# ZikangXiong/mobrob

Hardware: AMD Instinct MI355X
Metric: env-steps/sec (whole node), doggo PPO (higher is better)
Workload: dtype f32

## Files before the change

include/mobrob_ppo.h:

```cpp
#ifndef MOBROB_PPO_H
#define MOBROB_PPO_H

#include <stddef.h>
#include <stdint.h>

#ifdef __cplusplus
extern "C" {
#endif

#define MOBROB_PPO_ABI_VERSION 3
enum { MOBROB_ACT_TANH = 0, MOBROB_ACT_RELU = 1, MOBROB_ACT_ELU = 2, MOBROB_ACT_LEAKY_RELU = 3, MOBROB_ACT_SIGMOID = 4,
       MOBROB_ACT_SOFTPLUS = 5, MOBROB_ACT_SOFTSIGN = 6, MOBROB_ACT_HARDTANH = 7, MOBROB_ACT_RELU6 = 8, MOBROB_ACT_SILU = 9,
       MOBROB_ACT_GELU = 10, MOBROB_ACT_MISH = 11, MOBROB_ACT_COUNT = 12 };

enum {
  MOBROB_OK = 0,
  MOBROB_ERR_INVALID = -1,
  MOBROB_ERR_HIP = -2,
  MOBROB_ERR_STATE = -3,
  MOBROB_ERR_NO_DEVICE = -4
};

typedef struct mobrob_ppo_engine mobrob_ppo_engine_t;

// ... 459 lines not shown
  MOBROB_BUF_TERMINAL_OBS = 15,
  MOBROB_BUF_TERMINAL_VALUES = 16,
  MOBROB_BUF_TRUNCATED = 17,
  MOBROB_BUF_ENV_STATE = 18,
  MOBROB_BUF_GRAD_EXCHANGE = 19,
  MOBROB_BUF_SDE_NOISE = 20,
  MOBROB_BUF_COUNT = 21
};
int mobrob_ppo_buffer_info(mobrob_ppo_engine_t* e, int32_t which, void** ptr_dev, size_t* bytes);
int mobrob_ppo_read_buffer(mobrob_ppo_engine_t* e, int32_t which, void* host_out, size_t bytes);
int mobrob_ppo_write_buffer(mobrob_ppo_engine_t* e, int32_t which, const void* host_in, size_t bytes);
int mobrob_ppo_mark_rollout_ready(mobrob_ppo_engine_t* e);

int mobrob_ppo_x3_mode(const mobrob_ppo_engine_t* e);
int mobrob_ppo_update_mode(const mobrob_ppo_engine_t* e);

int mobrob_ppo_explained_variance(mobrob_ppo_engine_t* e, double* out);

int mobrob_ppo_compute_gae(mobrob_ppo_engine_t* e);

int mobrob_ppo_feistel_permutation(mobrob_ppo_engine_t* e, int64_t n, uint64_t key, int64_t* out);

enum {
  MOBROB_K_ACT = 0,
  MOBROB_K_GAE = 1,
  MOBROB_K_TRAIN_GRAD = 2,
  MOBROB_K_APPLY = 3,
  MOBROB_K_ENV = 4,
  MOBROB_K_GRAD_REDUCE = 5,
  MOBROB_K_ALLREDUCE = 6,
// ... 10 lines not shown
```

mobrob_amd/_lib.py:

```python
from __future__ import annotations

import ctypes as C
import os

_HERE = os.path.dirname(os.path.abspath(__file__))
LIB_PATH = os.environ.get("MOBROB_PPO_LIB") or os.path.join(_HERE, "libmobrob_ppo.so")
ABI_VERSION = 3

OK, ERR_INVALID, ERR_HIP, ERR_STATE, ERR_NO_DEVICE = 0, -1, -2, -3, -4

BUF = dict(obs=0, actions=1, rewards=2, episode_starts=3, values=4, log_probs=5, advantages=6, returns=7,
           params=8, grads=9, advstat=10, last_values=11, last_dones=12, clipped_actions=13, episode_start_state=14,
           terminal_obs=15, terminal_values=16, truncated=17, env_state=18, grad_exchange=19, sde_noise=20)
HYPER = dict(learning_rate=0, clip_range=1, clip_range_vf=2, target_kl=3, ent_coef=4, vf_coef=5, epoch_kernel=6)
KERNEL_IDS = dict(act=0, gae=1, train_grad=2, apply=3, env=4, grad_reduce=5, allreduce=6)


class Config(C.Structure):
    _fields_ = [
        ("abi_version", C.c_int32), ("obs_dim", C.c_int32), ("act_dim", C.c_int32),
        ("pi_hidden", C.c_int32 * 2), ("vf_hidden", C.c_int32 * 2),
        ("n_envs", C.c_int32), ("n_steps", C.c_int32), ("batch_size", C.c_int32), ("n_epochs", C.c_int32),
        ("gamma", C.c_double), ("gae_lambda", C.c_double), ("clip_range", C.c_double), ("ent_coef", C.c_double),
        ("vf_coef", C.c_double), ("max_grad_norm", C.c_double), ("learning_rate", C.c_double),
# ... 216 lines not shown
                                                   C.POINTER(C.c_uint16), C.c_int32, C.POINTER(C.c_int32), C.c_int32, _U8,
                                                   C.POINTER(C.c_int32), C.POINTER(C.c_int32)]),
    "mobrob_ppo_plan_assign": (C.c_int, [_P, C.POINTER(PlanSpec), C.POINTER(WallsC), C.POINTER(HazardsC), C.POINTER(HazardFramesC),
                                         C.POINTER(PlanTime), C.c_int32, C.c_int32, _F, _F, C.POINTER(C.c_int32), _F, C.POINTER(C.c_int32),
                                         _I64, C.POINTER(C.c_int32), _I64, _I64, C.POINTER(C.c_int32), C.POINTER(C.c_int32)]),
    "mobrob_ppo_sde_reset_noise": (C.c_int, [_P]),
    "mobrob_ppo_sde_set_noise": (C.c_int, [_P, _F]),
    "mobrob_ppo_buffer_info": (C.c_int, [_P, C.c_int32, C.POINTER(_P), C.POINTER(C.c_size_t)]),
    "mobrob_ppo_read_buffer": (C.c_int, [_P, C.c_int32, _P, C.c_size_t]),
    "mobrob_ppo_write_buffer": (C.c_int, [_P, C.c_int32, _P, C.c_size_t]),
    "mobrob_ppo_mark_rollout_ready": (C.c_int, [_P]),
    "mobrob_ppo_compute_gae": (C.c_int, [_P]),
    "mobrob_ppo_explained_variance": (C.c_int, [_P, C.POINTER(C.c_double)]),
    "mobrob_ppo_x3_mode": (C.c_int, [_P]),
    "mobrob_ppo_update_mode": (C.c_int, [_P]),
    "mobrob_ppo_feistel_permutation": (C.c_int, [_P, C.c_int64, C.c_uint64, _I64]),
    "mobrob_ppo_profile_enable": (C.c_int, [_P, C.c_int32]),
    "mobrob_ppo_profile_read": (C.c_int, [_P, C.POINTER(C.c_double), _I64]),
}

ALLREDUCE_FN = C.CFUNCTYPE(C.c_int, C.c_void_p, C.c_void_p, C.c_size_t, C.c_int32, C.c_void_p)

_lib = None


class EngineError(RuntimeError):
    pass


def load():
# ... 24 lines not shown
```

mobrob_amd/csrc/engine.hip:

```cpp
#include <hip/hip_runtime.h>
#include <rccl/rccl.h>
#include <dlfcn.h>

#include <algorithm>
#include <atomic>
#include <thread>
#include <cmath>
#include <cstdarg>
#include <cstdio>
#include <climits>
#include <cstring>
#include <ctime>
#include <cstdlib>
#include <string>
#include <vector>

#ifdef MOBROB_POISON_LDS
namespace mobrob {
__global__ __launch_bounds__(1024) void k_poison_lds() {
  extern __shared__ unsigned poison_words[];
  volatile unsigned* w = poison_words;
  for (int i = threadIdx.x; i < 160 * 256; i += 1024) w[i] = 0xFFFFFFFFu;
}
inline void poison_lds(hipStream_t st) {
// ... 158 lines not shown
  ncclComm_t comm = nullptr;
  int64_t allreduce_calls = 0, allreduce_bytes = 0;
  struct OneShot {
    char* xbuf = nullptr;
    size_t payload = 0;
    char* peer[kOneShotMaxRanks] = {nullptr};
    int world = 0, rank = -1;
    bool ready = false;
    unsigned long long seq = 0;
    int* error = nullptr;
    long long timeout_ticks = 0;
  } oneshot;
  double* norm_rec_sum = nullptr; int* norm_rec_t = nullptr; int* fold_idx_dev = nullptr;
  int fold_start[kMaxTensors + 1] = {0};
  bool use_norm_records = false;
  bool epoch_kernel_on = true;
  unsigned* epoch_bar = nullptr;
  float* epoch_consts = nullptr;
  int* epoch_idx = nullptr;
  char* epoch_stage = nullptr;
  int* epoch_err_host = nullptr;
  hipEvent_t epoch_ev = nullptr;
  int last_update_mode = 0;
  float* epoch_snap = nullptr;
  int rollout64_tile_max = 256;
  int pair64_min_tiles = 65;
  int split64_max_tiles = 64;
  float *Xg = nullptr, *actg = nullptr, *lpg = nullptr, *advg = nullptr, *retg = nullptr, *oldvg = nullptr;
  float *hp[kMaxHidden] = {nullptr}, *hv[kMaxHidden] = {nullptr}, *mu = nullptr, *vout = nullptr;
  float *dmu = nullptr, *dv = nullptr, *dzp[kMaxHidden] = {nullptr}, *dzv[kMaxHidden] = {nullptr};
// ... 43 lines not shown
  bool plan_clear_lds_set = false;
  char* plan_time_buf = nullptr;
  size_t plan_time_bytes = 0;
  bool plan_time_lds_set = false;
  char* plan_team_buf = nullptr;
  size_t plan_team_bytes = 0;
  bool plan_team_lds_set = false;
  bool plan_team_smooth_lds_set = false;
  bool plan_team_rounds_lds_set = false;
  bool plan_assign_lds_set = false;
};

namespace {

int check_async_error(mobrob_ppo_engine* e);

constexpr size_t kArenaAlign = 256;

template <typename Tp>
int dalloc(mobrob_ppo_engine* e, Tp** p, size_t count) {
  const size_t bytes = (std::max<size_t>(count, 1) * sizeof(Tp) + kArenaAlign - 1) / kArenaAlign * kArenaAlign;
  if (e->plan_only) {
    e->arena_used += bytes;
    *p = nullptr;
    return MOBROB_OK;
  }
  if (e->arena_used + bytes > e->arena_bytes)
    return fail(MOBROB_ERR_INVALID, "device arena too small: need more than %zu bytes", e->arena_bytes);
  void* q = e->arena + e->arena_used;
  e->arena_used += bytes;
// ... 199 lines not shown
    c.D = e->D; c.Dp = e->Dp;
    hipLaunchKernelGGL(k_pack_chain, dim3(FH * FH / 256, 2), dim3(256), 0, e->stream, c);
  }
}

void repack(mobrob_ppo_engine* e) {
  auto pad = [&](const float* src, float* dst, int r, int c, int rp, int cp) {
    hipLaunchKernelGGL(k_pad_rows, dim3(cdiv(rp * cp, 256)), dim3(256), 0, e->stream, src, dst, r, c, rp, cp);
  };
  pad(Pp(e, T_PW1), e->pW1p, e->H1, e->D, e->H1, e->Dp);
  pad(Pp(e, T_VW1), e->vW1p, e->G1, e->D, e->G1, e->Dp);
  pad(Pp(e, T_AW), e->aWp, e->A, e->HL, e->Ap, e->HL);
  pad(Pp(e, T_VW), e->vWp, 1, e->GL, 8, e->GL);
  fused_repack(e->fused, e->params, e->offs, e->stream);
  pack_x3_all(e);
}

void forward_generic(mobrob_ppo_engine* e, const float* X, int rows, bool want_pi, float* mu_out, bool want_v,
                     float* v_out, bool keep_z = false) {
  GemmQueue qp, qv;
  if (want_pi) {
    linear_fwd(e, X, e->Dp, e->pW1p, e->Dp, Pp(e, e->tPB[0]), e->hp[0], e->Hp[0], rows, e->Hp[0], e->Dp, true, keep_z ? e->dzp[0] : nullptr, &qp);
    for (int l = 1; l < e->Lp; ++l)
      linear_fwd(e, e->hp[l - 1], e->Hp[l - 1], Pp(e, e->tPW[l]), e->Hp[l - 1], Pp(e, e->tPB[l]), e->hp[l], e->Hp[l], rows, e->Hp[l], e->Hp[l - 1], true,
                 keep_z ? e->dzp[l] : nullptr, &qp);
    linear_fwd(e, e->hp[e->Lp - 1], e->HL, e->aWp, e->HL, Pp(e, T_AB), mu_out, e->Ap, rows, e->A, e->HL, false, nullptr, &qp);
  }
  if (want_v) {
    linear_fwd(e, X, e->Dp, e->vW1p, e->Dp, Pp(e, e->tVB[0]), e->hv[0], e->Hv[0], rows, e->Hv[0], e->Dp, true, keep_z ? e->dzv[0] : nullptr, &qv);
    for (int l = 1; l < e->Lv; ++l)
      linear_fwd(e, e->hv[l - 1], e->Hv[l - 1], Pp(e, e->tVW[l]), e->Hv[l - 1], Pp(e, e->tVB[l]), e->hv[l], e->Hv[l], rows, e->Hv[l], e->Hv[l - 1], true,
                 keep_z ? e->dzv[l] : nullptr, &qv);
    linear_fwd(e, e->hv[e->Lv - 1], e->GL, e->vWp, e->GL, Pp(e, T_VB), v_out, 1, rows, 1, e->GL, false, nullptr, &qv);
  }
  run_queues(e, qp, qv, 1);
}

void forward(mobrob_ppo_engine* e, const float* X, int rows, bool want_pi, float* mu_out, bool want_v, float* v_out) {
  if (e->fused.enabled && fused_forward(e->fused, X, rows, want_pi, mu_out, e->Ap, want_v, v_out, e->stream)) return;
  forward_generic(e, X, rows, want_pi, mu_out, want_v, v_out);
}

int value_net_width_sum(const mobrob_ppo_engine* e) {
  int s = 0;
  for (int l = 0; l < e->Lv; ++l) s += e->Hv[l];
  return s;
}
ValueNetArgs value_net_args(mobrob_ppo_engine* e) {
  ValueNetArgs vn{};
  for (int l = 0; l < e->Lv; ++l) { vn.W[l] = Pp(e, e->tVW[l]); vn.b[l] = Pp(e, e->tVB[l]); vn.G[l] = e->Hv[l]; }
  vn.Wv = Pp(e, T_VW); vn.bv = Pp(e, T_VB);
  vn.L = e->Lv; vn.act = e->cfg.activation; vn.width_sum = value_net_width_sum(e);
  return vn;
// ... 19 lines not shown
void sde_resample(mobrob_ppo_engine* e, int r0, int n, uint32_t draw, const uint32_t* draw_base, bool single) {
  const int HLA = e->HL * e->A, per = cdiv(HLA, 4);
  hipLaunchKernelGGL(k_sde_resample, dim3(cdiv((n + (single ? 1 : 0)) * per, 256)), dim3(256), 0, e->stream, Pp(e, T_LOGSTD), HLA, e->A, e->sde_mode, r0, n,
                     eps_seed(e) ^ 0x5DE5DE5DE5DE5DEull, draw, draw_base, e->sde_E, single ? e->sde_E1 : (float*)nullptr);
}

void sde_variance(mobrob_ppo_engine* e, int rows, bool fresh_table, float* lat2 = nullptr) {
  if (fresh_table)
    hipLaunchKernelGGL(k_sde_std2, dim3(cdiv(e->HL * e->A, 256)), dim3(256), 0, e->stream, Pp(e, T_LOGSTD), e->HL, e->A, e->sde_mode, e->sde_S2);
  hipLaunchKernelGGL(k_sde_var, dim3(cdiv(rows, 4)), dim3(256), 0, e->stream, e->hp[e->Lp - 1], e->HL, e->sde_S2, rows, e->HL, e->A, e->sde_var, e->Ap,
                     lat2);
}

void act_rows(mobrob_ppo_engine* e, int t, int r0, int n, const float* eps_dev_or_null, uint32_t draw,
              const uint32_t* draw_base, float* clip_out = nullptr) {
  ProfScope ps(e, MOBROB_K_ACT);
  if (!clip_out) clip_out = e->clip_act + (size_t)r0 * e->A;
  const size_t row = (size_t)t * e->N + r0;
  const float* X = e->obs + row * e->Dp;
  if (e->fused.enabled) {
    FusedActArgs a{};
    a.X = X; a.rows = n; a.row0 = r0; a.want_pi = 1; a.want_v = 1; a.mu = nullptr; a.ldmu = e->Ap;
    a.v = e->values + row; a.sample = 1; a.A = e->A; a.log_std = Pp(e, T_LOGSTD); a.eps = eps_dev_or_null;
    a.seed = eps_seed(e); a.draw = draw; a.draw_base = draw_base; a.lo = (float)e->cfg.action_low; a.hi = (float)e->cfg.action_high;
    a.act_raw = e->actions + row * e->A; a.act_clip = clip_out; a.logp = e->logp + row;
    fused_launch_act(e->fused, a, e->stream);
    return;
  }
  forward(e, X, n, true, e->mu, true, e->values + row);
  if (e->sde) {
// ... 62 lines not shown
StatsArgs stats_args(const mobrob_ppo_engine* e) {
  StatsArgs st{};
  st.loss_sums = e->grads + e->P; st.log_std = e->params + e->offs[T_LOGSTD]; st.n_act = e->A; st.sde = e->sde;
  st.ent_coef = (float)e->cfg.ent_coef; st.vf_coef = (float)e->cfg.vf_coef;
  return st;
}
int fused_carve_packs(mobrob_ppo_engine* e) {
  FusedState& f = e->fused;
  const int H = f.H;
  const size_t nW1 = (size_t)(H / 32) * (e->Dp / 8) * 256, nW2 = (size_t)(H / 32) * (H / 8) * 256;
  const size_t nW3f = (size_t)(H / 8) * 256, nW3b = (size_t)(H / 32) * 4 * 256;
  const size_t nW3h = (size_t)(H / 16) * 256;
  const size_t per_net = nW1 + 2 * nW2 + nW3f + nW3h + nW3b + 2 * H;
  f.packed_floats = 2 * per_net;
  CHK(dalloc(e, &f.packed, f.packed_floats));
  const int head_bias[2] = {T_AB, T_VB};
  for (int n = 0; n < 2; ++n) {
    float* p = f.packed + n * per_net;
    f.net[n].W1f = reinterpret_cast<const f32x4*>(p); p += nW1;
    f.net[n].W2f = reinterpret_cast<const f32x4*>(p); p += nW2;
    f.net[n].W3f = reinterpret_cast<const f32x4*>(p); p += nW3f;
    f.net[n].W2b = reinterpret_cast<const f32x4*>(p); p += nW2;
    f.net[n].W3b = reinterpret_cast<const f32x4*>(p); p += nW3b;
    f.net[n].b1s = p; p += H;
    f.net[n].b2s = p; p += H;
    f.net[n].W3h = reinterpret_cast<const f32x4*>(p); p += nW3h;
    f.net[n].b3 = e->params + e->offs[head_bias[n]];
    f.net[n].head = n == 0 ? e->A : 1;
    f.net[n].W1x = nullptr; f.net[n].W2x = nullptr; f.net[n].W2bx = nullptr;
    f.net[n].W1c = nullptr; f.net[n].W2c = nullptr; f.net[n].W2bc = nullptr; f.net[n].W3c = nullptr; f.net[n].W3bc = nullptr;
// ... 13 lines not shown
    f.lds_act_bytes = fused64_lds_bytes(e->Dp);
    CHK(dalloc(e, &e->epoch_bar, 1024));
    CHK(dalloc(e, &e->epoch_snap, (size_t)3 * e->P));
    CHK(dalloc(e, &e->epoch_consts, (size_t)2 * e->nmb));
    CHK(dalloc(e, &e->epoch_idx, (size_t)e->nmb));
  } else {
    f.slab_floats = slab_size(e->Dp);
    CHK(dalloc(e, &f.slabs, (size_t)f.max_grid * f.slab_floats));
    if (e->cfg.forward_x3 && e->cfg.activation == MOBROB_ACT_TANH && !env_switched_off("MOBROB_NO_X3")) {
      for (int n = 0; n < 2; ++n) {
        unsigned* w1 = nullptr; unsigned* w2 = nullptr; unsigned* w2b = nullptr;
        CHK(dalloc(e, &w1, (size_t)(H / 32) * (e->Dp / 16) * 192 * 4));
        CHK(dalloc(e, &w2, (size_t)(H / 32) * (H / 16) * 192 * 4));
        CHK(dalloc(e, &w2b, (size_t)(H / 32) * (H / 16) * 192 * 4));
        f.net[n].W1x = w1; f.net[n].W2x = w2; f.net[n].W2bx = w2b;
      }
      f.train_x3 = e->A <= 16 && e->Dp != 48 && !env_switched_off("MOBROB_NO_TRAIN_X3");
      f.train_chain = f.train_x3 && !env_switched_off("MOBROB_NO_CHAIN");
      if (f.train_chain) {
        const int K1 = (e->Dp + 31) / 32;
        for (int n = 0; n < 2; ++n) {
          unsigned* w1 = nullptr; unsigned* w2 = nullptr; unsigned* w2b = nullptr; float* w3 = nullptr; float* w3b = nullptr;
          CHK(dalloc(e, &w1, (size_t)K1 * 16 * 768));
          CHK(dalloc(e, &w2, (size_t)8 * 16 * 768));
          CHK(dalloc(e, &w2b, (size_t)8 * 16 * 768));
          CHK(dalloc(e, &w3, (size_t)16 * 64 * 4));
          CHK(dalloc(e, &w3b, (size_t)16 * 64 * 4));
          f.net[n].W1c = w1; f.net[n].W2c = w2; f.net[n].W2bc = w2b; f.net[n].W3c = w3; f.net[n].W3bc = w3b;
        }
        f.lds_chain_bytes = chain_lds_bytes(e->Dp);
      }
    }
    CHK(dalloc(e, &f.train_rec, (size_t)e->N * e->T * train_rec_width(e->A)));
    f.lds_bytes = fused_lds_bytes(e->Dp);
    f.lds_act_bytes = fused_lds_act_bytes(e->Dp);
  }
  return dalloc(e, &f.stamps, 32);
}
int build_norm_record_tables(mobrob_ppo_engine* e) {
  const FusedState& f = e->fused;
  const int nb = cdiv(f.slab_floats, 256);
  CHK(dalloc(e, &e->norm_rec_sum, (size_t)2 * nb * kNormRec));
  CHK(dalloc(e, &e->norm_rec_t, (size_t)2 * nb * kNormRec));
// ... 353 lines not shown
  e->stats_cap = std::max(64, 4 * e->nmb * cfg->n_epochs);
  e->chunk_table.clear();
  for (int tt = 0; tt < e->ntens; ++tt)
    for (int s0 = e->offs[tt]; s0 < e->offs[tt + 1]; s0 += 4096)
      e->chunk_table.push_back(NormChunk{tt, s0, std::min(s0 + 4096, e->offs[tt + 1]), 0});
  e->nchunks = (int)e->chunk_table.size();
  if (e->nchunks > 256) return fail(MOBROB_ERR_INVALID, "parameter vector too large for the norm chunk table (%d chunks)", e->nchunks);
  return MOBROB_OK;
}

int engine_alloc(mobrob_ppo_engine* e) {
  const size_t P = e->P, N = e->N, T = e->T, Dp = e->Dp, A = e->A, Bl = std::min(e->Bl, e->N * e->T), R = e->rows_max;
  CHK(dalloc(e, &e->params, P)); CHK(dalloc(e, &e->grads, P + 8)); CHK(dalloc(e, &e->m, P)); CHK(dalloc(e, &e->v, P));
  CHK(dalloc(e, &e->pW1p, (size_t)e->H1 * Dp)); CHK(dalloc(e, &e->vW1p, (size_t)e->G1 * Dp));
  CHK(dalloc(e, &e->aWp, (size_t)e->Ap * e->HL)); CHK(dalloc(e, &e->vWp, (size_t)8 * e->GL));
  CHK(dalloc(e, &e->obs, (T + 1) * N * Dp)); CHK(dalloc(e, &e->actions, T * N * A));
  CHK(dalloc(e, &e->rewards, T * N)); CHK(dalloc(e, &e->es, T * N)); CHK(dalloc(e, &e->values, (T + 1) * N));
  e->last_values = e->values + T * N;
  CHK(dalloc(e, &e->logp, T * N)); CHK(dalloc(e, &e->adv, T * N)); CHK(dalloc(e, &e->ret, T * N));
  CHK(dalloc(e, &e->last_dones, N)); CHK(dalloc(e, &e->prev_dones, N));
  CHK(dalloc(e, &e->dones_tmp, N)); CHK(dalloc(e, &e->clip_act, N * A)); CHK(dalloc(e, &e->rew_tmp, N));
  CHK(dalloc(e, &e->term_obs, N * Dp)); CHK(dalloc(e, &e->term_val, N)); CHK(dalloc(e, &e->eps_dev, R * A));
  CHK(dalloc(e, &e->trunc_dev, N)); CHK(dalloc(e, &e->dones_u8, N)); CHK(dalloc(e, &e->ep_len, N)); CHK(dalloc(e, &e->ep_len2, N)); CHK(dalloc(e, &e->ctr_dev, 2));
  CHK(dalloc(e, &e->rows, T * N)); CHK(dalloc(e, &e->perm_dev, T * N)); CHK(dalloc(e, &e->advstat, (size_t)e->nmb * 4)); CHK(dalloc(e, &e->advbins, (size_t)e->nmb * 2 + 1)); CHK(dalloc(e, &e->expvar_part, (size_t)kEvBlocks * 4));
  CHK(dalloc(e, &e->stats, (size_t)e->stats_cap * 8));
  CHK(dalloc(e, &e->Xg, Bl * Dp)); CHK(dalloc(e, &e->actg, Bl * A)); CHK(dalloc(e, &e->lpg, Bl));
  CHK(dalloc(e, &e->advg, Bl)); CHK(dalloc(e, &e->retg, Bl)); CHK(dalloc(e, &e->oldvg, Bl));
  for (int l = 0; l < e->Lp; ++l) CHK(dalloc(e, &e->hp[l], R * e->Hp[l]));
  for (int l = 0; l < e->Lv; ++l) CHK(dalloc(e, &e->hv[l], R * e->Hv[l]));
  CHK(dalloc(e, &e->mu, R * e->Ap)); CHK(dalloc(e, &e->vout, R));
// ... 419 lines not shown

int mobrob_ppo_compute_gae(mobrob_ppo_engine_t* e) {
  if (!e) return fail(MOBROB_ERR_INVALID, "null engine");
  run_gae(e);
  HIPC(hipStreamSynchronize(e->stream));
  e->rollout_ready = true; e->train_rec_valid = false;
  return MOBROB_OK;
}

int mobrob_ppo_x3_mode(const mobrob_ppo_engine_t* e) {
  if (!e || !e->fused.enabled || e->fused.net[0].W2x == nullptr) return 0;
  return 1 | (e->fused.train_x3 ? 2 : 0) | (e->fused.train_x3 && e->fused.train_chain ? 4 : 0);
}

int mobrob_ppo_update_mode(const mobrob_ppo_engine_t* e) { return e ? e->last_update_mode : 0; }

int mobrob_ppo_explained_variance(mobrob_ppo_engine_t* e, double* out) {
  if (!e || !out) return fail(MOBROB_ERR_INVALID, "explained_variance: null argument");
  if (!e->rollout_ready) return fail(MOBROB_ERR_STATE, "explained_variance: rollout not finished");
  const int n = e->N * e->T;
  hipLaunchKernelGGL(k_explained_variance_partials, dim3(kEvBlocks), dim3(256), 0, e->stream, e->values, e->ret, n, e->expvar_part);
  double part[kEvBlocks * 4];
  HIPC(hipMemcpyAsync(part, e->expvar_part, sizeof part, hipMemcpyDeviceToHost, e->stream));
  HIPC(hipStreamSynchronize(e->stream));
  double s[4] = {0.0, 0.0, 0.0, 0.0};
  for (int b = 0; b < kEvBlocks; ++b)
    for (int k = 0; k < 4; ++k) s[k] += part[b * 4 + k];
  const double var_y = s[1] / n - (s[0] / n) * (s[0] / n), var_d = s[3] / n - (s[2] / n) * (s[2] / n);
  *out = var_y > 0.0 ? 1.0 - var_d / var_y : NAN;
  return MOBROB_OK;
// ... 46 lines not shown
bool rollout_s8(const mobrob_ppo_engine* e) {
  static const bool s8_on = !kRolloutStationary && env_int("MOBROB_ROLLOUT_S8", 1) != 0;
  return s8_on && e->fused.net[0].W2x != nullptr;
}

struct ChunkPlan {
  bool overlap;
  int chunk, vgrid_max;
};
ChunkPlan chunk_plan(bool wide, int tiles, bool tile_kernel, int T, int N) {
  const bool overlap = tiles <= 192 && (wide || (tile_kernel && (size_t)T * N >= ((size_t)1 << 18)));
  return ChunkPlan{overlap, overlap ? std::max(16, cdiv(T, 20)) : T, overlap ? std::max(32, 256 - tiles) : 256};
}

void launch_rollout_kernel(mobrob_ppo_engine* e, const RolloutArgs& a) {
  const int Dp = e->Dp, tiles = cdiv(a.N, 32);
  if (!wide_nets(e)) {
    if (a.kind == 3) {
      FUSED_DISPATCH_DP(Dp, hipLaunchKernelGGL((k_rollout64_tile<DPc, 3>), dim3(tiles), dim3(256), rollout64_tile_lds_bytes(Dp, true), e->stream, a));
    } else if (rollout64_tile_kernel(e)) {
      FUSED_DISPATCH_DP(Dp, hipLaunchKernelGGL((k_rollout64_tile<DPc>), dim3(tiles), dim3(256), rollout64_tile_lds_bytes(Dp), e->stream, a));
    } else {
      const int nwv = rollout64_waves(Dp);
      FUSED_DISPATCH_DP(Dp, hipLaunchKernelGGL((k_rollout64_persistent<DPc>), dim3(cdiv(tiles, nwv)), dim3(nwv * 64), rollout64_lds_bytes(Dp), e->stream, a));
    }
    return;
  }
  const bool s8 = a.kind == 3 || rollout_s8(e);
  const dim3 grid(tiles), block(kRolloutThreads);
  const size_t lds = rollout_lds_bytes(Dp, s8);
// ... 639 lines not shown
    a.fW3b[n] = on && !ch ? (float*)e->fused.net[n].W3b : nullptr;
    a.fW3h[n] = (on && (n == 1 || e->fused.A <= 16)) ? (float*)e->fused.net[n].W3h : nullptr;
    a.fb1s[n] = on ? (float*)e->fused.net[n].b1s : nullptr;
    a.fb2s[n] = on ? (float*)e->fused.net[n].b2s : nullptr;
    const bool x3 = on && e->fused.train_x3;
    a.xW1[n] = x3 ? reinterpret_cast<unsigned short*>(const_cast<unsigned*>(e->fused.net[n].W1x)) : nullptr;
    a.xW2[n] = x3 ? reinterpret_cast<unsigned short*>(const_cast<unsigned*>(e->fused.net[n].W2x)) : nullptr;
    a.xW2b[n] = x3 && !ch ? reinterpret_cast<unsigned short*>(const_cast<unsigned*>(e->fused.net[n].W2bx)) : nullptr;
    a.cW1[n] = ch ? reinterpret_cast<unsigned short*>(const_cast<unsigned*>(e->fused.net[n].W1c)) : nullptr;
    a.cW2[n] = ch ? reinterpret_cast<unsigned short*>(const_cast<unsigned*>(e->fused.net[n].W2c)) : nullptr;
    a.cW2b[n] = ch ? reinterpret_cast<unsigned short*>(const_cast<unsigned*>(e->fused.net[n].W2bc)) : nullptr;
    a.cW3[n] = ch ? const_cast<float*>(e->fused.net[n].W3c) : nullptr;
    a.cW3b[n] = ch ? const_cast<float*>(e->fused.net[n].W3bc) : nullptr;
  }
}
}

namespace {
struct AdamStep { float step_size, bc2_sqrt; };
AdamStep next_adam_step(mobrob_ppo_engine* e) {
  e->adam_step++;
  const double bc1 = 1.0 - std::pow(e->cfg.adam_beta1, (double)e->adam_step), bc2 = 1.0 - std::pow(e->cfg.adam_beta2, (double)e->adam_step);
  return {(float)(e->cfg.learning_rate / bc1), (float)std::sqrt(bc2)};
}
int next_stats_row(mobrob_ppo_engine* e) {
  if (e->stats_n >= e->stats_cap) e->stats_n = 0;
  return e->stats_n++;
}
StatsArgs apply_norms(mobrob_ppo_engine* e) {
  StatsArgs st = stats_args(e);
  st.stats_row = e->stats + (size_t)next_stats_row(e) * 8;
  st.inv_bg = 1.0f / (float)((int64_t)e->cur_count * e->cfg.world_size);
  if (!e->use_norm_records)
    hipLaunchKernelGGL(k_sqnorm_chunks, dim3(e->nchunks), dim3(256), 0, e->stream, e->grads, e->chunks_dev,
                       e->chunk_partial, st);
  return st;
}
int apply_adam(mobrob_ppo_engine* e, const StatsArgs& st) {
  const AdamStep step = next_adam_step(e);
  AdamPackArgs a{};
  fill_adam_pack_args(e, a);
  a.step_size = step.step_size; a.bc2_sqrt = step.bc2_sqrt;
  if (e->use_norm_records) a.st = st;
  a.stats_row = st.stats_row;
  a.loss_sums_zero = e->fused.enabled ? e->grads + e->P : nullptr;
  hipLaunchKernelGGL(k_adam_pack, dim3(cdiv(e->P, 256)), dim3(256), 0, e->stream, a);
  HIPC(hipGetLastError());
  e->grad_pending = false;
  return MOBROB_OK;
}
}

namespace {
int apply_checked(mobrob_ppo_engine* e, int32_t* stopped) {
  *stopped = 0;
  ProfScope ps(e, MOBROB_K_APPLY);
  const StatsArgs st = apply_norms(e);
  if (e->target_kl > 0.0) {
    float approx_kl = 0.f;
    HIPC(hipMemcpyAsync(&approx_kl, st.stats_row + 4, sizeof(float), hipMemcpyDeviceToHost, e->stream));
// ... 256 lines not shown
}

int train_loop(mobrob_ppo_engine* e, const int64_t* perms, bool dp, bool records, mobrob_allreduce_fn fn, void* ctx) {
  if (!dp && e->cfg.world_size != 1)
    return fail(MOBROB_ERR_STATE, "mobrob_ppo_train is the single-rank loop; data-parallel ranks call mobrob_ppo_train_dp "
                                  "(or drive epoch_begin/minibatch_grad/[all-reduce]/minibatch_apply)");
  const size_t total = (size_t)e->N * e->T;
  e->stats_n = 0;
  const bool kl = e->target_kl > 0.0;
  e->last_epochs_started = 0; e->last_stopped_early = 0; e->last_steps_applied = 0;
  struct RecordsOn {
    mobrob_ppo_engine* e;
    RecordsOn(mobrob_ppo_engine* e_, bool on) : e(e_) { e->use_norm_records = on; }
    ~RecordsOn() { e->use_norm_records = false; }
  } records_on(e, records);
  EpochLaunch epoch_launch;
  const bool epoch_kernel = epoch_kernel_eligible(e, dp, records, &epoch_launch);
  e->last_update_mode = epoch_kernel ? 1 : 0;
  for (int ep = 0; ep < e->cfg.n_epochs; ++ep) {
    CHK(mobrob_ppo_epoch_begin(e, perms ? perms + (size_t)ep * total : nullptr));
    if (dp) CHK(dp_all_reduce(e, e->advstat, (size_t)e->nmb * 4, 1, fn, ctx));
    e->last_epochs_started = ep + 1;
    if (ep == e->cfg.n_epochs - 1 || kl) e->stats_n = 0;
    if (epoch_kernel) {
      CHK(launch_epoch_kernel(e, ep, epoch_launch));
      continue;
    }
    for (int mb = 0; mb < e->nmb && !e->last_stopped_early; ++mb) {
      CHK(mobrob_ppo_minibatch_grad(e, mb));
      if (dp) CHK(dp_all_reduce(e, e->grads, (size_t)e->P + 8, 0, fn, ctx));
// ... 2370 lines not shown
```

mobrob_amd/csrc/kernels_fused.h:

```cpp
#pragma once
#include "device_utils.h"

namespace mobrob {

constexpr int FH = 256;
constexpr int FR = 64;
constexpr int FLDH = FH + 4;
constexpr int FLDO = 36;
constexpr int FTHREADS = 256;

struct FusedNet {
  const f32x4* W1f;
  const f32x4* W2f;
  const f32x4* W3f;
  const f32x4* W3h;
  const f32x4* W2b;
  const f32x4* W3b;
  const float* b1s; const float* b2s;
  const float* b3;
  int head;
  const unsigned* W1x;
  const unsigned* W2x;
  const unsigned* W2bx;
  const unsigned* W1c;
// ... 1908 lines not shown
  out[base + 1024] = (unsigned short)(p3 & 0xffffu);
}
__device__ __forceinline__ void chain_store_w1(unsigned short* w1c, int n, int k, int K1, float scaled) {
  chain_pack_store(w1c, chain_pack_idx(chain_unit_w1(n >> 4, k >> 5, K1), n, (k >> 3) & 3, k & 7), scaled);
}
__device__ __forceinline__ void chain_store_w2(unsigned short* w2c, unsigned short* w2bc, int n, int k, float scaled, float raw) {
  int s, g, j;
  chain_kslot_of_neuron(k, &s, &g, &j);
  chain_pack_store(w2c, chain_pack_idx(chain_unit_w2(n >> 4, s), n, g, j), scaled);
  chain_kslot_of_neuron(n, &s, &g, &j);
  chain_pack_store(w2bc, chain_pack_idx(chain_unit_w2b(k >> 4, s), k, g, j), raw);
}
__host__ __device__ __forceinline__ int chain_head_fwd_idx(int a_, int k) { return ((k >> 4) * 64 + a_ + 16 * ((k >> 2) & 3)) * 4 + (k & 3); }
__host__ __device__ __forceinline__ int chain_head_bwd_idx(int a_, int k) { return ((k >> 4) * 64 + (k & 15) + 16 * (a_ >> 2)) * 4 + (a_ & 3); }

template <bool COH = false, class TA = AdamPackArgs>
__device__ __forceinline__ void adam_pack_apply(const TA& a, int i, float graw, float m0, float v0, float p0, float coef, float step_size, float bc2_sqrt) {
  const float g = __fmul_rn(graw, coef);
  const float m = __fmaf_rn(g, 1.0f - a.beta1, __fmul_rn(m0, a.beta1));
  const float v = __fmaf_rn(__fmul_rn(g, g), 1.0f - a.beta2, __fmul_rn(v0, a.beta2));
  const float denom = __fadd_rn(__fdiv_rn(__fsqrt_rn(v), bc2_sqrt), a.eps);
  const float pn = __fmaf_rn(-step_size, __fdiv_rn(m, denom), p0);
  int t = 0;
#pragma unroll
  for (int k = 1; k < kFusedTensors; ++k) t += (i >= a.offs[k]) ? 1 : 0;
  if (a.ntens > kFusedTensors)
    for (int k = kFusedTensors; k < a.ntens; ++k) t += (i >= a.offs[k]) ? 1 : 0;
  const int e = i - a.offs[t];
  a.m[i] = m;
  a.v[i] = v;
  if (COH && a.two_by_two && (t == 0 || t == 10 || t == 12)) stc<true>(a.p + i, pn);
  else a.p[i] = pn;
#ifdef ADAM_NO_PACK
  return;
#endif
  if (!a.two_by_two) {
    if (t == a.id_pw1 || t == a.id_vw1) {
      const int n = e / a.D, k = e - n * a.D;
      (t == a.id_vw1 ? a.vW1p : a.pW1p)[n * a.Dp + k] = pn;
    } else if (t == a.id_aw || t == a.id_vw) {
      (t == a.id_vw ? a.vWp : a.aWp)[e] = pn;
    }
    return;
  }
  switch (t) {
    case 1: case 5: {
      const int net = t == 5, n = e / a.D, k = e - n * a.D;
      (net ? a.vW1p : a.pW1p)[n * a.Dp + k] = pn;
      if (a.fW1f[net]) stc<COH>(a.fW1f[net] + pack_fwd_idx(n, k, a.Dp / 8), kTanhScale * pn);
      if (a.xW1[net]) x3_pack_store(a.xW1[net], n, k, a.Dp / 16, kTanhScale * pn);
      if (a.cW1[net]) chain_store_w1(a.cW1[net], n, k, (a.Dp + 31) / 32, kTanhScale * pn);
    } break;
    case 3: case 7: {
      const int net = t == 7;
      if (a.fW2f[net]) {
        const int K = net ? a.G1 : a.H1, n = e / K, k = e - n * K;
        stc<COH>(a.fW2f[net] + pack_fwd_idx(n, k, K / 8), kTanhScale * pn);
        if (a.fW2b[net]) stc<COH>(a.fW2b[net] + pack_bwd_idx(n, k, (net ? a.G2 : a.H2) / 8), pn);
        if (a.xW2[net]) x3_pack_store(a.xW2[net], n, k, K / 16, kTanhScale * pn);
        if (a.xW2b[net]) x3_pack_store(a.xW2b[net], k, n, (net ? a.G2 : a.H2) / 16, pn);
        if (a.cW2[net]) chain_store_w2(a.cW2[net], a.cW2b[net], n, k, kTanhScale * pn, pn);
      }
    } break;
    case 9: case 11: {
      const int net = t == 11, K = net ? a.G2 : a.H2, n = e / K, k = e - n * K;
      (net ? a.vWp : a.aWp)[e] = pn;
      if (a.fW3f[net]) {
        stc<COH>(a.fW3f[net] + pack_fwd_idx(n, k, K / 8), pn);
        if (a.fW3b[net]) stc<COH>(a.fW3b[net] + pack_bwd_idx(n, k, 4), pn);
        if (a.fW3h[net] && n < 16) stc<COH>(a.fW3h[net] + pack_h16_idx(n, k), pn);
        if (a.cW3[net] && n < 16) { a.cW3[net][chain_head_fwd_idx(n, k)] = pn; a.cW3b[net][chain_head_bwd_idx(n, k)] = pn; }
      }
    } break;
    case 2: case 6: if (a.fb1s[t == 6]) stc<COH>(a.fb1s[t == 6] + e, kTanhScale * pn); break;
    case 4: case 8: if (a.fb2s[t == 8]) stc<COH>(a.fb2s[t == 8] + e, kTanhScale * pn); break;
    default: break;
  }
}

template <bool COH, class TA>
__device__ __forceinline__ void adam_pack_block_at(const TA& a, int lin, int i, float g_in, float m_in, float v_in, float p_in, float step_size,
                                                   float bc2_sqrt, float* stats_row, float inv_bg, float ent_pre, int fidx_pre = -1) {
  __shared__ double part[1024];
  __shared__ int tens[256];
  __shared__ float nts[kMaxTensors + 3];
  __shared__ float coef_s, total_s;
  if (lin == 0 && a.st.loss_sums != nullptr) {
    StatsArgs st;
    st.stats_row = stats_row; st.loss_sums = a.st.loss_sums; st.log_std = a.st.log_std;
    st.ent_coef = a.st.ent_coef; st.vf_coef = a.st.vf_coef; st.inv_bg = inv_bg; st.n_act = a.st.n_act; st.sde = a.st.sde;
    stats_row_from_sums<COH>(st, ent_pre);
  }
// ... 50 lines not shown
  if (lin == 0 && stats_row != nullptr) stats_row[6] = total_s;
  if (lin < 8 && a.loss_sums_zero != nullptr) stc<COH>(a.loss_sums_zero + lin, 0.f);
  if (i < 0 || i >= a.P) return;
  adam_pack_apply<COH>(a, i, g_in, m_in, v_in, p_in, coef, step_size, bc2_sqrt);
}
template <bool COH, class TA>
__device__ __forceinline__ void adam_pack_block(const TA& a, int bx, float step_size, float bc2_sqrt, float* stats_row, float inv_bg) {
  const int i = bx * 256 + (int)threadIdx.x;
  float g_in = 0.f, m_in = 0.f, v_in = 0.f, p_in = 0.f;
  if (i < a.P) { g_in = ldc<COH>(a.g + i); m_in = ldc<COH>(a.m + i); v_in = ldc<COH>(a.v + i); p_in = ldc<COH>(a.p + i); }
  const float ent = (i == 0 && a.st.loss_sums != nullptr) ? entropy_of_log_std<COH>(a.st.log_std, a.st.n_act) : 0.f;
  adam_pack_block_at<COH>(a, i, i, g_in, m_in, v_in, p_in, step_size, bc2_sqrt, stats_row, inv_bg, ent);
}
__global__ __launch_bounds__(256) void k_adam_pack(AdamPackArgs a) {
  adam_pack_block<false>(a, blockIdx.x, a.step_size, a.bc2_sqrt, a.stats_row, a.st.inv_bg);
}

struct FusedState {
  bool enabled = false;
  int H = 0;
  int D = 0, Dp = 0, A = 0;
  float* packed = nullptr;
  size_t packed_floats = 0;
  FusedNet net[2];
  float* slabs = nullptr;
  float* train_rec = nullptr;
  bool train_x3 = false;
  bool train_chain = false;
  size_t lds_chain_bytes = 0;
  unsigned long long* stamps = nullptr;
// ... 55 lines not shown
```

mobrob_amd/engine.py:

```python
from __future__ import annotations

import ctypes as C
from collections import OrderedDict

import numpy as np

from . import _lib
from ._lib import BUF, Config, DroneParams, EpisodeStats, EvalSpec, FollowSpec, GoalEnv, HazardFramesC, HazardsC, TrainStats, check

F32 = np.float32
STAT_KEYS = ("policy_loss", "value_loss", "entropy_loss", "loss", "approx_kl", "clip_fraction", "grad_norm")


def _fp(a):
    return None if a is None else a.ctypes.data_as(C.POINTER(C.c_float))


def _u8(a):
    return None if a is None else a.ctypes.data_as(C.POINTER(C.c_uint8))


def _f32c(a, shape=None):
    a = np.ascontiguousarray(a, dtype=F32)
    if shape is not None and a.shape != tuple(shape):
# ... 1026 lines not shown
            raise ValueError("pos, rpy, goal must be [n, 3] and action [n, 18]")
        if ctrl_state.shape != (n, 12) or ctrl_state.dtype != F32 or not ctrl_state.flags.c_contiguous:
            raise ValueError("ctrl_state must be a C-contiguous float32 [n, 12] array")
        prm = DroneParams(mass, g, dt, max_thrust, max_xy_torque, max_z_torque, max_roll_pitch, tune_fac)
        out = np.empty((n, 4), F32)
        check(self.lib.mobrob_ctrl_drone_pid(self._h, n, 0, C.byref(prm), _fp(pos), _fp(rpy), _fp(goal), _fp(action),
                                             _fp(ctrl_state), _fp(out)))
        return out

    def compute_gae(self):
        check(self.lib.mobrob_ppo_compute_gae(self._h))

    def x3_mode(self):
        return int(self.lib.mobrob_ppo_x3_mode(self._h))

    def update_mode(self):
        return int(self.lib.mobrob_ppo_update_mode(self._h))

    def explained_variance(self):
        out = C.c_double()
        check(self.lib.mobrob_ppo_explained_variance(self._h, C.byref(out)))
        return float(out.value)

    def mark_rollout_ready(self):
        check(self.lib.mobrob_ppo_mark_rollout_ready(self._h))

    def train(self, perms=None):
        p = None
        if perms is not None:
            perms = np.ascontiguousarray(perms, dtype=np.int64)
# ... 225 lines not shown
```

Baseline: 32.35 million.

## Defer rollout weight packing until after the final Adam step of training

During training with the fused chain path, each Adam step now writes only the training-side packed weight layouts and marks the rollout-side packs stale. A separate pack-only kernel rebuilds the forward/x3 packs once, either lazily before the next forward or rollout launch or when training ends. This removes redundant scattered stores to rollout layouts on every minibatch step. In exchange it adds an extra kernel launch per update and staleness bookkeeping. A read_packs API is also added so the packed buffers can be inspected.

```diff
diff --git a/include/mobrob_ppo.h b/include/mobrob_ppo.h
--- a/include/mobrob_ppo.h
+++ b/include/mobrob_ppo.h
@@ -497,6 +497,7 @@
 
 int mobrob_ppo_x3_mode(const mobrob_ppo_engine_t* e);
 int mobrob_ppo_update_mode(const mobrob_ppo_engine_t* e);
+int64_t mobrob_ppo_read_packs(mobrob_ppo_engine_t* e, void* out, int64_t capacity);
 
 int mobrob_ppo_explained_variance(mobrob_ppo_engine_t* e, double* out);
 
diff --git a/mobrob_amd/_lib.py b/mobrob_amd/_lib.py
--- a/mobrob_amd/_lib.py
+++ b/mobrob_amd/_lib.py
@@ -254,6 +254,7 @@
     "mobrob_ppo_explained_variance": (C.c_int, [_P, C.POINTER(C.c_double)]),
     "mobrob_ppo_x3_mode": (C.c_int, [_P]),
     "mobrob_ppo_update_mode": (C.c_int, [_P]),
+    "mobrob_ppo_read_packs": (C.c_int64, [_P, C.c_void_p, C.c_int64]),
     "mobrob_ppo_feistel_permutation": (C.c_int, [_P, C.c_int64, C.c_uint64, _I64]),
     "mobrob_ppo_profile_enable": (C.c_int, [_P, C.c_int32]),
     "mobrob_ppo_profile_read": (C.c_int, [_P, C.POINTER(C.c_double), _I64]),
diff --git a/mobrob_amd/csrc/engine.hip b/mobrob_amd/csrc/engine.hip
--- a/mobrob_amd/csrc/engine.hip
+++ b/mobrob_amd/csrc/engine.hip
@@ -196,6 +196,9 @@
   double* norm_rec_sum = nullptr; int* norm_rec_t = nullptr; int* fold_idx_dev = nullptr;
   int fold_start[kMaxTensors + 1] = {0};
   bool use_norm_records = false;
+  bool defer_packs = false;
+  bool rollout_packs_stale = false;
+  std::vector<std::pair<const void*, size_t>> pack_segments;
   bool epoch_kernel_on = true;
   unsigned* epoch_bar = nullptr;
   float* epoch_consts = nullptr;
@@ -269,6 +272,7 @@
 namespace {
 
 int check_async_error(mobrob_ppo_engine* e);
+int ensure_rollout_packs(mobrob_ppo_engine* e);
 
 constexpr size_t kArenaAlign = 256;
 
@@ -498,6 +502,7 @@
   pad(Pp(e, T_VW), e->vWp, 1, e->GL, 8, e->GL);
   fused_repack(e->fused, e->params, e->offs, e->stream);
   pack_x3_all(e);
+  e->rollout_packs_stale = false;
 }
 
 void forward_generic(mobrob_ppo_engine* e, const float* X, int rows, bool want_pi, float* mu_out, bool want_v,
@@ -521,6 +526,7 @@
 }
 
 void forward(mobrob_ppo_engine* e, const float* X, int rows, bool want_pi, float* mu_out, bool want_v, float* v_out) {
+  (void)ensure_rollout_packs(e);
   if (e->fused.enabled && fused_forward(e->fused, X, rows, want_pi, mu_out, e->Ap, want_v, v_out, e->stream)) return;
   forward_generic(e, X, rows, want_pi, mu_out, want_v, v_out);
 }
@@ -570,6 +576,7 @@
 
 void act_rows(mobrob_ppo_engine* e, int t, int r0, int n, const float* eps_dev_or_null, uint32_t draw,
               const uint32_t* draw_base, float* clip_out = nullptr) {
+  (void)ensure_rollout_packs(e);
   ProfScope ps(e, MOBROB_K_ACT);
   if (!clip_out) clip_out = e->clip_act + (size_t)r0 * e->A;
   const size_t row = (size_t)t * e->N + r0;
@@ -662,6 +669,7 @@
   const size_t per_net = nW1 + 2 * nW2 + nW3f + nW3h + nW3b + 2 * H;
   f.packed_floats = 2 * per_net;
   CHK(dalloc(e, &f.packed, f.packed_floats));
+  e->pack_segments.push_back({f.packed, f.packed_floats * 4});
   const int head_bias[2] = {T_AB, T_VB};
   for (int n = 0; n < 2; ++n) {
     float* p = f.packed + n * per_net;
@@ -705,6 +713,9 @@
         CHK(dalloc(e, &w2, (size_t)(H / 32) * (H / 16) * 192 * 4));
         CHK(dalloc(e, &w2b, (size_t)(H / 32) * (H / 16) * 192 * 4));
         f.net[n].W1x = w1; f.net[n].W2x = w2; f.net[n].W2bx = w2b;
+        e->pack_segments.push_back({w1, (size_t)(H / 32) * (e->Dp / 16) * 192 * 4 * 4});
+        e->pack_segments.push_back({w2, (size_t)(H / 32) * (H / 16) * 192 * 4 * 4});
+        e->pack_segments.push_back({w2b, (size_t)(H / 32) * (H / 16) * 192 * 4 * 4});
       }
       f.train_x3 = e->A <= 16 && e->Dp != 48 && !env_switched_off("MOBROB_NO_TRAIN_X3");
       f.train_chain = f.train_x3 && !env_switched_off("MOBROB_NO_CHAIN");
@@ -718,6 +729,11 @@
           CHK(dalloc(e, &w3, (size_t)16 * 64 * 4));
           CHK(dalloc(e, &w3b, (size_t)16 * 64 * 4));
           f.net[n].W1c = w1; f.net[n].W2c = w2; f.net[n].W2bc = w2b; f.net[n].W3c = w3; f.net[n].W3bc = w3b;
+          e->pack_segments.push_back({w1, (size_t)K1 * 16 * 768 * 4});
+          e->pack_segments.push_back({w2, (size_t)8 * 16 * 768 * 4});
+          e->pack_segments.push_back({w2b, (size_t)8 * 16 * 768 * 4});
+          e->pack_segments.push_back({w3, (size_t)16 * 64 * 4 * 4});
+          e->pack_segments.push_back({w3b, (size_t)16 * 64 * 4 * 4});
         }
         f.lds_chain_bytes = chain_lds_bytes(e->Dp);
       }
@@ -1101,6 +1117,7 @@
   CHK(dalloc(e, &e->params, P)); CHK(dalloc(e, &e->grads, P + 8)); CHK(dalloc(e, &e->m, P)); CHK(dalloc(e, &e->v, P));
   CHK(dalloc(e, &e->pW1p, (size_t)e->H1 * Dp)); CHK(dalloc(e, &e->vW1p, (size_t)e->G1 * Dp));
   CHK(dalloc(e, &e->aWp, (size_t)e->Ap * e->HL)); CHK(dalloc(e, &e->vWp, (size_t)8 * e->GL));
+  e->pack_segments = {{e->pW1p, (size_t)e->H1 * Dp * 4}, {e->vW1p, (size_t)e->G1 * Dp * 4}, {e->aWp, (size_t)e->Ap * e->HL * 4}, {e->vWp, (size_t)8 * e->GL * 4}};
   CHK(dalloc(e, &e->obs, (T + 1) * N * Dp)); CHK(dalloc(e, &e->actions, T * N * A));
   CHK(dalloc(e, &e->rewards, T * N)); CHK(dalloc(e, &e->es, T * N)); CHK(dalloc(e, &e->values, (T + 1) * N));
   e->last_values = e->values + T * N;
@@ -1550,6 +1567,20 @@
 }
 
 int mobrob_ppo_update_mode(const mobrob_ppo_engine_t* e) { return e ? e->last_update_mode : 0; }
+int64_t mobrob_ppo_read_packs(mobrob_ppo_engine_t* e, void* out, int64_t capacity) {
+  if (!e) return fail(MOBROB_ERR_INVALID, "null engine");
+  size_t total = 0;
+  for (const auto& sg : e->pack_segments) total += sg.second;
+  if (!out) return (int64_t)total;
+  if (capacity < (int64_t)total) return fail(MOBROB_ERR_INVALID, "read_packs: %lld bytes given, %zu needed", (long long)capacity, total);
+  size_t at = 0;
+  for (const auto& sg : e->pack_segments) {
+    HIPC(hipMemcpyAsync(static_cast<char*>(out) + at, sg.first, sg.second, hipMemcpyDeviceToHost, e->stream));
+    at += sg.second;
+  }
+  HIPC(hipStreamSynchronize(e->stream));
+  return (int64_t)total;
+}
 
 int mobrob_ppo_explained_variance(mobrob_ppo_engine_t* e, double* out) {
   if (!e || !out) return fail(MOBROB_ERR_INVALID, "explained_variance: null argument");
@@ -1626,6 +1657,7 @@
 }
 
 void launch_rollout_kernel(mobrob_ppo_engine* e, const RolloutArgs& a) {
+  (void)ensure_rollout_packs(e);
   const int Dp = e->Dp, tiles = cdiv(a.N, 32);
   if (!wide_nets(e)) {
     if (a.kind == 3) {
@@ -2295,6 +2327,28 @@
     a.cW3b[n] = ch ? const_cast<float*>(e->fused.net[n].W3bc) : nullptr;
   }
 }
+void select_rollout_packs(AdamPackArgs& a, bool keep) {
+  for (int n = 0; n < 2; ++n) {
+    if (!keep) {
+      a.fW1f[n] = a.fW2f[n] = a.fW3f[n] = a.fW3h[n] = nullptr;
+      a.xW1[n] = a.xW2[n] = nullptr;
+    } else {
+      a.fW2b[n] = a.fW3b[n] = a.fb1s[n] = a.fb2s[n] = nullptr;
+      a.xW2b[n] = a.cW1[n] = a.cW2[n] = a.cW2b[n] = nullptr;
+      a.cW3[n] = a.cW3b[n] = nullptr;
+    }
+  }
+}
+int ensure_rollout_packs(mobrob_ppo_engine* e) {
+  if (!e->rollout_packs_stale) return MOBROB_OK;
+  AdamPackArgs a{};
+  fill_adam_pack_args(e, a);
+  select_rollout_packs(a, true);
+  hipLaunchKernelGGL(k_pack_only, dim3(cdiv(e->P, 256)), dim3(256), 0, e->stream, a);
+  HIPC(hipGetLastError());
+  e->rollout_packs_stale = false;
+  return MOBROB_OK;
+}
 }
 
 namespace {
@@ -2325,6 +2379,10 @@
   if (e->use_norm_records) a.st = st;
   a.stats_row = st.stats_row;
   a.loss_sums_zero = e->fused.enabled ? e->grads + e->P : nullptr;
+  if (e->defer_packs) {
+    select_rollout_packs(a, false);
+    e->rollout_packs_stale = true;
+  }
   hipLaunchKernelGGL(k_adam_pack, dim3(cdiv(e->P, 256)), dim3(256), 0, e->stream, a);
   HIPC(hipGetLastError());
   e->grad_pending = false;
@@ -2611,6 +2669,16 @@
     RecordsOn(mobrob_ppo_engine* e_, bool on) : e(e_) { e->use_norm_records = on; }
     ~RecordsOn() { e->use_norm_records = false; }
   } records_on(e, records);
+  struct LeanTail {
+    mobrob_ppo_engine* e;
+    explicit LeanTail(mobrob_ppo_engine* e_) : e(e_) {
+      e->defer_packs = e->fused.enabled && e->fused.train_chain && !env_switched_off("MOBROB_NO_LEAN_TAIL");
+    }
+    ~LeanTail() {
+      e->defer_packs = false;
+      (void)ensure_rollout_packs(e);
+    }
+  } lean_tail(e);
   EpochLaunch epoch_launch;
   const bool epoch_kernel = epoch_kernel_eligible(e, dp, records, &epoch_launch);
   e->last_update_mode = epoch_kernel ? 1 : 0;
diff --git a/mobrob_amd/csrc/kernels_fused.h b/mobrob_amd/csrc/kernels_fused.h
--- a/mobrob_amd/csrc/kernels_fused.h
+++ b/mobrob_amd/csrc/kernels_fused.h
@@ -1946,26 +1946,18 @@
 __host__ __device__ __forceinline__ int chain_head_fwd_idx(int a_, int k) { return ((k >> 4) * 64 + a_ + 16 * ((k >> 2) & 3)) * 4 + (k & 3); }
 __host__ __device__ __forceinline__ int chain_head_bwd_idx(int a_, int k) { return ((k >> 4) * 64 + (k & 15) + 16 * (a_ >> 2)) * 4 + (a_ & 3); }
 
-template <bool COH = false, class TA = AdamPackArgs>
-__device__ __forceinline__ void adam_pack_apply(const TA& a, int i, float graw, float m0, float v0, float p0, float coef, float step_size, float bc2_sqrt) {
-  const float g = __fmul_rn(graw, coef);
-  const float m = __fmaf_rn(g, 1.0f - a.beta1, __fmul_rn(m0, a.beta1));
-  const float v = __fmaf_rn(__fmul_rn(g, g), 1.0f - a.beta2, __fmul_rn(v0, a.beta2));
-  const float denom = __fadd_rn(__fdiv_rn(__fsqrt_rn(v), bc2_sqrt), a.eps);
-  const float pn = __fmaf_rn(-step_size, __fdiv_rn(m, denom), p0);
+template <class TA>
+__device__ __forceinline__ int adam_tensor_of(const TA& a, int i) {
   int t = 0;
 #pragma unroll
   for (int k = 1; k < kFusedTensors; ++k) t += (i >= a.offs[k]) ? 1 : 0;
   if (a.ntens > kFusedTensors)
     for (int k = kFusedTensors; k < a.ntens; ++k) t += (i >= a.offs[k]) ? 1 : 0;
+  return t;
+}
+template <bool COH, class TA>
+__device__ __forceinline__ void adam_pack_scatter(const TA& a, int i, int t, float pn) {
   const int e = i - a.offs[t];
-  a.m[i] = m;
-  a.v[i] = v;
-  if (COH && a.two_by_two && (t == 0 || t == 10 || t == 12)) stc<true>(a.p + i, pn);
-  else a.p[i] = pn;
-#ifdef ADAM_NO_PACK
-  return;
-#endif
   if (!a.two_by_two) {
     if (t == a.id_pw1 || t == a.id_vw1) {
       const int n = e / a.D, k = e - n * a.D;
@@ -1984,30 +1976,42 @@
       if (a.cW1[net]) chain_store_w1(a.cW1[net], n, k, (a.Dp + 31) / 32, kTanhScale * pn);
     } break;
     case 3: case 7: {
-      const int net = t == 7;
-      if (a.fW2f[net]) {
-        const int K = net ? a.G1 : a.H1, n = e / K, k = e - n * K;
-        stc<COH>(a.fW2f[net] + pack_fwd_idx(n, k, K / 8), kTanhScale * pn);
-        if (a.fW2b[net]) stc<COH>(a.fW2b[net] + pack_bwd_idx(n, k, (net ? a.G2 : a.H2) / 8), pn);
-        if (a.xW2[net]) x3_pack_store(a.xW2[net], n, k, K / 16, kTanhScale * pn);
-        if (a.xW2b[net]) x3_pack_store(a.xW2b[net], k, n, (net ? a.G2 : a.H2) / 16, pn);
-        if (a.cW2[net]) chain_store_w2(a.cW2[net], a.cW2b[net], n, k, kTanhScale * pn, pn);
-      }
+      const int net = t == 7, K = net ? a.G1 : a.H1, n = e / K, k = e - n * K;
+      if (a.fW2f[net]) stc<COH>(a.fW2f[net] + pack_fwd_idx(n, k, K / 8), kTanhScale * pn);
+      if (a.fW2b[net]) stc<COH>(a.fW2b[net] + pack_bwd_idx(n, k, (net ? a.G2 : a.H2) / 8), pn);
+      if (a.xW2[net]) x3_pack_store(a.xW2[net], n, k, K / 16, kTanhScale * pn);
+      if (a.xW2b[net]) x3_pack_store(a.xW2b[net], k, n, (net ? a.G2 : a.H2) / 16, pn);
+      if (a.cW2[net]) chain_store_w2(a.cW2[net], a.cW2b[net], n, k, kTanhScale * pn, pn);
     } break;
     case 9: case 11: {
       const int net = t == 11, K = net ? a.G2 : a.H2, n = e / K, k = e - n * K;
       (net ? a.vWp : a.aWp)[e] = pn;
-      if (a.fW3f[net]) {
-        stc<COH>(a.fW3f[net] + pack_fwd_idx(n, k, K / 8), pn);
-        if (a.fW3b[net]) stc<COH>(a.fW3b[net] + pack_bwd_idx(n, k, 4), pn);
-        if (a.fW3h[net] && n < 16) stc<COH>(a.fW3h[net] + pack_h16_idx(n, k), pn);
-        if (a.cW3[net] && n < 16) { a.cW3[net][chain_head_fwd_idx(n, k)] = pn; a.cW3b[net][chain_head_bwd_idx(n, k)] = pn; }
-      }
+      if (a.fW3f[net]) stc<COH>(a.fW3f[net] + pack_fwd_idx(n, k, K / 8), pn);
+      if (a.fW3b[net]) stc<COH>(a.fW3b[net] + pack_bwd_idx(n, k, 4), pn);
+      if (a.fW3h[net] && n < 16) stc<COH>(a.fW3h[net] + pack_h16_idx(n, k), pn);
+      if (a.cW3[net] && n < 16) { a.cW3[net][chain_head_fwd_idx(n, k)] = pn; a.cW3b[net][chain_head_bwd_idx(n, k)] = pn; }
     } break;
     case 2: case 6: if (a.fb1s[t == 6]) stc<COH>(a.fb1s[t == 6] + e, kTanhScale * pn); break;
     case 4: case 8: if (a.fb2s[t == 8]) stc<COH>(a.fb2s[t == 8] + e, kTanhScale * pn); break;
     default: break;
   }
+}
+template <bool COH = false, class TA = AdamPackArgs>
+__device__ __forceinline__ void adam_pack_apply(const TA& a, int i, float graw, float m0, float v0, float p0, float coef, float step_size, float bc2_sqrt) {
+  const float g = __fmul_rn(graw, coef);
+  const float m = __fmaf_rn(g, 1.0f - a.beta1, __fmul_rn(m0, a.beta1));
+  const float v = __fmaf_rn(__fmul_rn(g, g), 1.0f - a.beta2, __fmul_rn(v0, a.beta2));
+  const float denom = __fadd_rn(__fdiv_rn(__fsqrt_rn(v), bc2_sqrt), a.eps);
+  const float pn = __fmaf_rn(-step_size, __fdiv_rn(m, denom), p0);
+  const int t = adam_tensor_of(a, i);
+  a.m[i] = m;
+  a.v[i] = v;
+  if (COH && a.two_by_two && (t == 0 || t == 10 || t == 12)) stc<true>(a.p + i, pn);
+  else a.p[i] = pn;
+#ifdef ADAM_NO_PACK
+  return;
+#endif
+  adam_pack_scatter<COH>(a, i, t, pn);
 }
 
 template <bool COH, class TA>
@@ -2088,6 +2092,11 @@
 }
 __global__ __launch_bounds__(256) void k_adam_pack(AdamPackArgs a) {
   adam_pack_block<false>(a, blockIdx.x, a.step_size, a.bc2_sqrt, a.stats_row, a.st.inv_bg);
+}
+__global__ __launch_bounds__(256) void k_pack_only(AdamPackArgs a) {
+  const int i = blockIdx.x * 256 + (int)threadIdx.x;
+  if (i >= a.P) return;
+  adam_pack_scatter<false>(a, i, adam_tensor_of(a, i), a.p[i]);
 }
 
 struct FusedState {
diff --git a/mobrob_amd/engine.py b/mobrob_amd/engine.py
--- a/mobrob_amd/engine.py
+++ b/mobrob_amd/engine.py
@@ -1064,6 +1064,13 @@
     def x3_mode(self):
         return int(self.lib.mobrob_ppo_x3_mode(self._h))
 
+    def read_packs(self):
+        n = int(self.lib.mobrob_ppo_read_packs(self._h, None, 0))
+        check(min(n, 0))
+        out = np.empty(n, np.uint8)
+        check(min(int(self.lib.mobrob_ppo_read_packs(self._h, out.ctypes.data, n)), 0))
+        return out
+
     def update_mode(self):
         return int(self.lib.mobrob_ppo_update_mode(self._h))
 
```

Result: no change. 32.45 million, median of 5 (+0.3%).
